# jpreprocess/jbonsai

Hardware: AMD Instinct MI355X
Metric: 48 kHz PCM samples/sec (whole node), batched utterances (higher is better)
Workload: dtype f64

## Files before the change

jbonsai_amd/csrc/jb_vocoder.hip:

```cpp
#include "jb_device.h"

#include <cstdlib>
#include <cstring>

namespace jb {

__global__ void k_pitch(BatchDev bd, VocDev vd)
{
    const int b = blockIdx.y;
    const UttDev *u = bd.utt + b;
    const uint32_t t = blockIdx.x * blockDim.x + threadIdx.x;
    if (t >= u->T)
        return;
    const uint64_t f = u->frame_off + t;
    const double MAX_LF0 = 9.903487552536127, MIN_LF0 = 2.995732273553991;
    auto pitch_of = [&](double l) {
        if (l == kNoData)
            return 0.0;
        const double cl = l < MIN_LF0 ? MIN_LF0 : (l > MAX_LF0 ? MAX_LF0 : l);
        return (double)vd.fs / exp(cl);
    };
    const double p = pitch_of(vd.lf0[f]);
    const double prevp = t > 0 ? pitch_of(vd.lf0[f - 1]) : 0.0;
    vd.pitch[f] = p;
// ... 479 lines not shown
    if (vd.pitch[f] != 0.0) {
        const unsigned long long pm = vd.pmask[f * (uint64_t)nblk + (uint64_t)(i / bs)];
        x = ((pm >> (i % bs)) & 1ull) ? sqrt(fma((double)i, vd.pinc[f], vd.cur_start[f])) : 0.0;
    } else {
        x = vd.noise[(uint64_t)vd.uv_before[f] * (uint64_t)fp + (uint64_t)i];
    }
    if (vd.exc)
        vd.exc[base * (uint64_t)fp + n] = x;
    vd.xin[base * (uint64_t)fp + n] = x;
}

constexpr int kExw = 4;
constexpr int kExwHalo = 32;
constexpr int kExwQ = (256 + kExwHalo) / kExw;

constexpr int kN4Group = 4;
template <int NLPF>
__device__ __forceinline__ bool exc_pulse_free(const VocDev &vd, const int fp, const long n0,
                                               const double *__restrict__ tc, const double *__restrict__ tpp,
                                               const bool vcur, const bool vprev, const int lane,
                                               double (*ec)[kExwQ], double *ep, double *xs, double (&x)[kExw])
{
    static_assert(NLPF - 1 <= kExwHalo - 2, "history window too short");
    constexpr int kExwWin = NLPF - 1 + kExw;
    constexpr int anti = (NLPF - 1) / 2;
    constexpr int HQ = kExwHalo / kExw;
    const int i0 = lane * kExw;
    const bool own = i0 < fp;
    double ck[NLPF];
#pragma unroll
    for (int k = 0; k < NLPF; k++)
        ck[k] = tc[k];
    const double tpv = lane < NLPF ? tpp[lane] : 0.0;
    const long nl = own ? n0 + i0 : n0;
    const double2 nva = *reinterpret_cast<const double2 *>(vd.noise + nl);
    const double2 nvb = *reinterpret_cast<const double2 *>(vd.noise + nl + 2);
    double xi[kExw];
#pragma unroll
    for (int r = 0; r < kExw; r++) {
        const long q = nl + r - anti;
        const double v = vd.noise[q < 0 ? 0 : q];
        xi[r] = q < 0 ? 0.0 : v;
    }
    const long nt = n0 - kExwHalo + i0;
    const bool has_tail = lane < HQ && nt >= 0;
    const long ntc = has_tail ? nt : n0;
    const double2 tla = *reinterpret_cast<const double2 *>(vd.noise + ntc);
    const double2 tlb = *reinterpret_cast<const double2 *>(vd.noise + ntc + 2);
    const double nv[kExw] = {nva.x, nva.y, nvb.x, nvb.y};
#pragma unroll
    for (int r = 0; r < kExw; r++)
        x[r] = xi[r];
    if (vcur) {
        if (lane < HQ) {
#pragma unroll
            for (int r = 0; r < kExw; r++)
                ec[r][lane] = 0.0;
        }
        if (own) {
#pragma unroll
            for (int r = 0; r < kExw; r++)
                ec[r][HQ + lane] = 0.0 - nv[r];
        }
    }
    if (vprev) {
        if (lane < HQ) {
            const double tl[kExw] = {tla.x, tla.y, tlb.x, tlb.y};
#pragma unroll
            for (int r = 0; r < kExw; r++)
                ep[i0 + r] = has_tail ? 0.0 - tl[r] : 0.0;
        } else if (lane < 2 * HQ) {
#pragma unroll
            for (int r = 0; r < kExw; r++)
                ep[i0 + r] = 0.0;
        }
    }
    __builtin_amdgcn_fence(__ATOMIC_RELEASE, "wavefront");
    __builtin_amdgcn_wave_barrier();
    __builtin_amdgcn_fence(__ATOMIC_ACQUIRE, "wavefront");
    if (vcur && own) {
        constexpr int G = kN4Group;
#pragma unroll
        for (int k0 = 0; k0 < NLPF; k0 += G) {
            const int k1 = k0 + G - 1 < NLPF - 1 ? k0 + G - 1 : NLPF - 1;
            const int lo = NLPF - 1 - k1;
            double wg[G + kExw - 1];
#pragma unroll
            for (int c = 0; c < G + kExw - 1; c++) {
                const int idx = lo + c;
                if (idx < kExwWin) {
                    if (idx >= NLPF - 1) {
                        wg[c] = 0.0 - nv[idx - (NLPF - 1)];
                    } else {
                        const int o = idx + kExwHalo - (NLPF - 1);
                        wg[c] = ec[o & (kExw - 1)][lane + (o >> 2)];
                    }
                } else {
                    wg[c] = 0.0;
                }
            }
#pragma unroll
            for (int k = k0; k <= k1; k++) {
#pragma unroll
                for (int r = 0; r < kExw; r++)
                    x[r] = fma(wg[NLPF - 1 + r - k - lo], ck[k], x[r]);
            }
        }
    }
    if (vprev) {
        if (own && i0 < kExwHalo) {
#pragma unroll
            for (int r = 0; r < kExw; r++)
                xs[i0 + r] = x[r];
        }
        __builtin_amdgcn_fence(__ATOMIC_RELEASE, "wavefront");
        __builtin_amdgcn_wave_barrier();
        __builtin_amdgcn_fence(__ATOMIC_ACQUIRE, "wavefront");
        {
            double tk[NLPF];
#pragma unroll
            for (int k = 1; k < NLPF; k++) {
                const int lo = __builtin_amdgcn_readlane(__double2loint(tpv), k);
                const int hi = __builtin_amdgcn_readlane(__double2hiint(tpv), k);
                tk[k] = __hiloint2double(hi, lo);
            }
            if (lane < NLPF - 1 && lane < fp) {
                double xv = xs[lane];
#pragma unroll
                for (int k = 1; k < NLPF; k++)
                    xv = fma(ep[lane - k + kExwHalo], tk[k], xv);
                xs[lane] = xv;
            }
        }
        __builtin_amdgcn_fence(__ATOMIC_RELEASE, "wavefront");
        __builtin_amdgcn_wave_barrier();
        __builtin_amdgcn_fence(__ATOMIC_ACQUIRE, "wavefront");
        if (own && i0 < kExwHalo) {
#pragma unroll
            for (int r = 0; r < kExw; r++)
                x[r] = xs[i0 + r];
        }
    }
    return own;
}

template <int NLPF>
__global__ __launch_bounds__(256) void k_exc_classify(BatchDev bd, VocDev vd)
{
    const int b = blockIdx.y;
    const UttDev *u = bd.utt + b;
    const int wv = threadIdx.x >> 6, lane = threadIdx.x & 63;
    const uint32_t T = u->T;
    const uint32_t fr0 = (blockIdx.x * 4u + (uint32_t)wv) * 64u;
    if (blockIdx.x * 256u >= T)
        return;
    __shared__ uint32_t wcount[4], wbase;
    const uint64_t base = u->frame_off;
    unsigned long long canon = 0ull;
    bool canon64 = false;
    if (!vd.exc_no_table && vd.lpf_canon) {
        const long fa = (long)fr0 - 1 + lane;
        const bool ina = fa >= 0 && fa < (long)T;
        const uint8_t ca = vd.lpf_canon[base + (uint64_t)(ina ? fa : 0)];
        const long fb = (long)fr0 + 63;
        const uint8_t cb = vd.lpf_canon[base + (uint64_t)(fb < (long)T ? fb : 0)];
        canon = __ballot(ina && ca != 0);
        canon64 = fb < (long)T && cb != 0;
    } else if (!vd.exc_no_table) {
        const int half = lane >> 5, k = lane & 31;
        const bool tap = k < NLPF;
        const double cref = vd.lpf[tap ? k : 0];
        double v[33];
#pragma unroll
        for (int s = 0; s < 33; s++) {
            const long fr = (long)fr0 - 1 + 2 * s + half;
            const bool in = tap && fr >= 0 && fr < (long)T;
            v[s] = vd.lpf[in ? (base + (uint64_t)fr) * (uint64_t)NLPF + (uint64_t)k : (uint64_t)(tap ? k : 0)];
            if (!(fr >= 0 && fr < (long)T))
                v[s] = __longlong_as_double(~__double_as_longlong(cref));
        }
#pragma unroll
        for (int s = 0; s < 33; s++)
            asm volatile("" : "+v"(v[s]));
#pragma unroll
        for (int s = 0; s < 33; s++) {
            const bool eq = !tap || __double_as_longlong(v[s]) == __double_as_longlong(cref);
            const unsigned long long m = __ballot(eq);
            const bool ea = (uint32_t)m == 0xFFFFFFFFu, eb = (uint32_t)(m >> 32) == 0xFFFFFFFFu;
            if (s < 32)
                canon |= ((unsigned long long)ea << (2 * s)) | ((unsigned long long)eb << (2 * s + 1));
            else
                canon64 = ea;
        }
    }
    const uint32_t fr = fr0 + (uint32_t)lane;
    const bool in = fr < T;
    const uint64_t f = base + (in ? fr : 0u);
    const bool vcur = in && vd.voiced[f] != 0;
    const bool vprev = in && fr > 0 && vd.voiced[f - 1] != 0;
    const bool ccur = lane == 63 ? canon64 : ((canon >> (lane + 1)) & 1ull) != 0;
    const bool cprev = ((canon >> lane) & 1ull) != 0;
    uint32_t code = 0;
    if (!vd.exc_no_table && !vcur && !vprev && fr >= 1)
        code = 1;
    else if (!vd.exc_no_table && vcur && vprev && ccur && cprev)
        code = 2;
    if (in)
        vd.exc_src[f] = (uint8_t)code;
    const bool gen = in && code == 0;
    const unsigned long long gm = __ballot(gen);
    if (lane == 0)
        wcount[wv] = (uint32_t)__popcll(gm);
    __syncthreads();
    if (threadIdx.x == 0) {
        const uint32_t tot = wcount[0] + wcount[1] + wcount[2] + wcount[3];
        wbase = tot ? atomicAdd(vd.exc_gen_count, tot) : 0u;
    }
    __syncthreads();
    uint32_t slot0 = wbase;
    for (int w = 0; w < wv; w++)
        slot0 += wcount[w];
    if (gen) {
        const uint32_t rank = (uint32_t)__popcll(gm & ((1ull << lane) - 1ull));
        uint32_t *e = vd.exc_gen + 2 * (uint64_t)(slot0 + rank);
        e[0] = (uint32_t)b;
        e[1] = fr | (vcur ? 1u << 30 : 0u) | (vprev ? 1u << 31 : 0u);
    }
}

template <int NLPF>
__global__ __launch_bounds__(256) void k_exc_table(BatchDev bd, VocDev vd)
{
    const int wv = threadIdx.x >> 6, lane = threadIdx.x & 63;
    const uint32_t fr = (uint32_t)__builtin_amdgcn_readfirstlane((int)(blockIdx.x * 4u + (uint32_t)wv));
    if (fr == 0 || fr >= bd.maxT)
        return;
    __shared__ double ec_s[4][kExw][kExwQ];
    __shared__ double ep_s[4][2 * kExwHalo];
    __shared__ double xs_s[4][kExwHalo];
    const int fp = vd.fperiod;
    const long n0 = (long)fr * (long)fp;
    double x[kExw];
    if (!exc_pulse_free<NLPF>(vd, fp, n0, vd.lpf, vd.lpf, true, true, lane, ec_s[wv], ep_s[wv], xs_s[wv], x))
        return;
    double *o = vd.exc_tab + (uint64_t)n0 + (uint64_t)(lane * kExw);
    *reinterpret_cast<double2 *>(o) = make_double2(x[0], x[1]);
    *reinterpret_cast<double2 *>(o + 2) = make_double2(x[2], x[3]);
}

template <int NLPF>
__global__ __launch_bounds__(256) void k_exc_general(BatchDev bd, VocDev vd)
{
    const int wv = threadIdx.x >> 6, lane = threadIdx.x & 63;
    __shared__ double ec_s[4][kExw][kExwQ];
    __shared__ double ep_s[4][2 * kExwHalo];
    __shared__ double xs_s[4][kExwHalo];
    const uint32_t count = *vd.exc_gen_count;
    const uint32_t stride = gridDim.x * 4u;
    uint32_t i = blockIdx.x * 4u + (uint32_t)wv;
    if (i >= count)
        return;
    const int fp = vd.fperiod;
    uint32_t eb = vd.exc_gen[2 * (uint64_t)i], ef = vd.exc_gen[2 * (uint64_t)i + 1];
    for (; i < count; i += stride) {
        const int b = __builtin_amdgcn_readfirstlane((int)eb);
        const uint32_t efu = (uint32_t)__builtin_amdgcn_readfirstlane((int)ef);
        const uint32_t inext = i + stride < count ? i + stride : i;
        eb = vd.exc_gen[2 * (uint64_t)inext];
        ef = vd.exc_gen[2 * (uint64_t)inext + 1];
        const uint32_t fr = efu & 0x3FFFFFFFu;
        const bool vcur = (efu >> 30 & 1u) != 0, vprev = (efu >> 31) != 0;
        const uint64_t base = bd.utt[b].frame_off;
        const uint64_t f = base + fr;
        const uint64_t fprev = fr > 0 ? f - 1 : f;
        const long n0 = (long)fr * (long)fp;
        double x[kExw];
        const bool own = exc_pulse_free<NLPF>(vd, fp, n0, lpf_row(vd, f, NLPF), lpf_row(vd, fprev, NLPF),
                                              vcur, vprev, lane, ec_s[wv], ep_s[wv], xs_s[wv], x);
        if (own) {
            const uint64_t o = base * (uint64_t)fp + (uint64_t)n0 + (uint64_t)(lane * kExw);
            *reinterpret_cast<double2 *>(vd.xin + o) = make_double2(x[0], x[1]);
            *reinterpret_cast<double2 *>(vd.xin + o + 2) = make_double2(x[2], x[3]);
            if (vd.exc) {
                *reinterpret_cast<double2 *>(vd.exc + o) = make_double2(x[0], x[1]);
                *reinterpret_cast<double2 *>(vd.exc + o + 2) = make_double2(x[2], x[3]);
            }
        }
        __builtin_amdgcn_fence(__ATOMIC_RELEASE, "wavefront");
        __builtin_amdgcn_wave_barrier();
        __builtin_amdgcn_fence(__ATOMIC_ACQUIRE, "wavefront");
    }
}

__device__ __forceinline__ double readlane_f64(double v, int lane)
{
    int lo = __builtin_amdgcn_readlane(__double2loint(v), lane);
    int hi = __builtin_amdgcn_readlane(__double2hiint(v), lane);
    return __hiloint2double(hi, lo);
}

constexpr int kFixFrames = 8;

template <int NLPF>
__global__ __launch_bounds__(256) void k_excite_fix(BatchDev bd, VocDev vd)
{
    const int b = blockIdx.y;
    const UttDev *u = bd.utt + b;
    const int wv = threadIdx.x >> 6, lane = threadIdx.x & 63;
    const uint32_t T = u->T;
    const uint64_t base = u->frame_off;
    const int fp = vd.fperiod, bs = vd.bs, nblk = vd.nblk;
    constexpr int H = NLPF - 1;
    __shared__ double tap_s[4][2][NLPF];
    double(*tap2)[NLPF] = tap_s[wv];
    static_assert(kFixFrames * 4 <= 32, "one lane per (frame, mask word), twice");
    const int s0 = lane * kExw;
    const bool own = s0 < fp;
    const bool blk_rows = bs % kExw == 0 && bs % 2 == 0 && nblk <= 4;
    int myblk = 0;
    for (int q = 1; q < nblk; q++)
        myblk += s0 >= q * bs ? 1 : 0;
    const int tail0 = fp - H;
    unsigned long long mword = 0ull;
    uint32_t vfl = 0, codev = 0;
    uint32_t cnv = 0;
    {
        const int half = lane >> 5, jf = (lane & 31) / 4, q = lane & 3;
        const long frl = (long)((blockIdx.x * (uint32_t)kFixFrames + (uint32_t)jf) * 4u + (uint32_t)wv) - half;
        if (frl >= 0 && frl < (long)T) {
            if (q == 0)
                vfl = vd.voiced[base + (uint64_t)frl];
            if (q == 1 && half == 0 && vd.exc_src)
                codev = vd.exc_src[base + (uint64_t)frl];
            if (q == 2 && vd.lpf_sparse)
                cnv = vd.lpf_canon[base + (uint64_t)frl];
            if (q < nblk)
                mword = vd.pmask[(base + (uint64_t)frl) * (uint64_t)nblk + (uint64_t)q];
        }
        const uint32_t vq = (uint32_t)__builtin_amdgcn_update_dpp(0, (int)vfl, 0x00, 0xf, 0xf, true);
        if (!vq)
            mword = 0ull;
        if (half) {
            const int qt = tail0 / bs, lo = tail0 - qt * bs;
            if (q < qt)
                mword = 0ull;
            else if (q == qt && lo > 0)
                mword &= ~0ull << lo;
        }
    }
    const unsigned long long nz = __ballot(mword != 0ull);
    auto words_of = [&](int jf) -> uint32_t {
        return (uint32_t)((nz >> (32 + 4 * jf)) & 0xFull) | ((uint32_t)((nz >> (4 * jf)) & 0xFull) << 4);
    };
    auto each_pulse = [&](int jf, uint32_t m8, auto fn) {
        while (m8) {
            const int idx = __builtin_ctz(m8);
            m8 &= m8 - 1u;
            const int ownf = idx >> 2, q = idx & 3;
            const int src = (ownf ? 0 : 32) + jf * 4 + q;
            const uint32_t wl = (uint32_t)__builtin_amdgcn_readlane((int)(uint32_t)mword, src);
            const uint32_t wh = (uint32_t)__builtin_amdgcn_readlane((int)(uint32_t)(mword >> 32), src);
            unsigned long long w = ((unsigned long long)wh << 32) | wl;
            while (w) {
                const int j = __builtin_ctzll(w);
                w &= w - 1ull;
                fn(ownf ? q * bs + j : q * bs + j - fp, ownf, q * bs + j);
            }
        }
    };
#ifndef JB_FIX_GROUP
#define JB_FIX_GROUP 4
#endif
    constexpr int kFixGroup = JB_FIX_GROUP;
    static_assert(kFixFrames % kFixGroup == 0, "whole groups");
    for (int j0 = 0; j0 < kFixFrames; j0 += kFixGroup) {
        bool work[kFixGroup], touched[kFixGroup], from_tab[kFixGroup];
        uint32_t bmask[kFixGroup];
        double tv[kFixGroup], pv[kFixGroup], x[kFixGroup][kExw];
#pragma unroll
        for (int g = 0; g < kFixGroup; g++) {
            const int jf = j0 + g;
            const uint32_t fr = (uint32_t)__builtin_amdgcn_readfirstlane(
                (int)((blockIdx.x * (uint32_t)kFixFrames + (uint32_t)jf) * 4u + (uint32_t)wv));
            work[g] = touched[g] = from_tab[g] = false;
            bmask[g] = 0;
            tv[g] = pv[g] = 0.0;
#pragma unroll
            for (int r = 0; r < kExw; r++)
                x[g][r] = 0.0;
            if (fr >= T)
                continue;
            const uint64_t f = base + fr;
            const uint32_t m8 = words_of(jf);
            if (!m8)
                continue;
            const bool any_p = (m8 & 0xFu) != 0, any_c = (m8 >> 4) != 0;
            bool tch = false;
            each_pulse(jf, m8, [&](int p, int, int) { tch = tch || (s0 + kExw - 1 >= p && s0 <= p + H); });
            from_tab[g] = (__builtin_amdgcn_readlane((int)codev, 4 * jf + 1) & 3) == 2;
            work[g] = true;
            bool in_blk = true;
            if (from_tab[g] && blk_rows) {
                uint32_t bm = 0;
                for (int q = 0; q < nblk; q++)
                    if (__ballot(tch && own && myblk == q))
                        bm |= 1u << q;
                bmask[g] = bm;
                in_blk = ((bm >> myblk) & 1u) != 0;
            }
            touched[g] = (tch || (from_tab[g] && in_blk)) && own;
            {
                const int hw = lane >> 5, k = lane & 31;
                const uint32_t cn_c = (uint32_t)__builtin_amdgcn_readlane((int)cnv, 4 * jf + 2);
                const uint32_t cn_p = (uint32_t)__builtin_amdgcn_readlane((int)cnv, 32 + 4 * jf + 2);
                if (k < NLPF && (hw ? any_c : any_p))
                    tv[g] = vd.lpf[((hw ? cn_c : cn_p) ? 0ull : f - 1 + (uint64_t)hw) * (uint64_t)NLPF + (uint64_t)k];
                if (lane < 4 && ((lane >> 1) ? any_c : any_p)) {
                    const uint64_t ff = f - 1 + (uint64_t)(lane >> 1);
                    pv[g] = (lane & 1) ? vd.pinc[ff] : vd.cur_start[ff];
                }
            }
            if (touched[g]) {
                const double *src = from_tab[g] ? vd.exc_tab + ((uint64_t)fr * (uint64_t)fp + (uint64_t)s0)
                                                : vd.xin + (f * (uint64_t)fp + (uint64_t)s0);
                const double2 xa = *reinterpret_cast<const double2 *>(src);
                const double2 xb = *reinterpret_cast<const double2 *>(src + 2);
                x[g][0] = xa.x;
                x[g][1] = xa.y;
                x[g][2] = xb.x;
                x[g][3] = xb.y;
            }
        }
#pragma unroll
        for (int g = 0; g < kFixGroup; g++) {
            if (!work[g])
                continue;
            const int jf = j0 + g;
            const uint32_t fr = (uint32_t)__builtin_amdgcn_readfirstlane(
                (int)((blockIdx.x * (uint32_t)kFixFrames + (uint32_t)jf) * 4u + (uint32_t)wv));
            const uint64_t f = base + fr;
            __builtin_amdgcn_fence(__ATOMIC_RELEASE, "wavefront");
            __builtin_amdgcn_wave_barrier();
            if ((lane & 31) < NLPF)
                tap2[lane >> 5][lane & 31] = tv[g];
            const double cs_p = readlane_f64(pv[g], 0), pi_p = readlane_f64(pv[g], 1);
            const double cs_c = readlane_f64(pv[g], 2), pi_c = readlane_f64(pv[g], 3);
            __builtin_amdgcn_fence(__ATOMIC_RELEASE, "wavefront");
            __builtin_amdgcn_wave_barrier();
            __builtin_amdgcn_fence(__ATOMIC_ACQUIRE, "wavefront");
            each_pulse(jf, words_of(jf), [&](int p, int gsel, int i) {
                const double amp = sqrt(gsel ? fma((double)i, pi_c, cs_c) : fma((double)i, pi_p, cs_p));
#pragma unroll
                for (int r = 0; r < kExw; r++) {
                    const int k = s0 + r - p;
                    const bool in = k >= 0 && k <= H;
                    const double tk = tap2[gsel][in ? k : 0];
                    if (in)
                        x[g][r] = fma(amp, tk, x[g][r]);
                }
            });
            if (touched[g]) {
                const uint64_t o = f * (uint64_t)fp + (uint64_t)s0;
                *reinterpret_cast<double2 *>(vd.xin + o) = make_double2(x[g][0], x[g][1]);
                *reinterpret_cast<double2 *>(vd.xin + o + 2) = make_double2(x[g][2], x[g][3]);
                if (vd.exc) {
                    *reinterpret_cast<double2 *>(vd.exc + o) = make_double2(x[g][0], x[g][1]);
                    *reinterpret_cast<double2 *>(vd.exc + o + 2) = make_double2(x[g][2], x[g][3]);
                }
            }
            if (from_tab[g] && lane == 0)
                vd.exc_src[f] = blk_rows ? (uint8_t)(2u | (bmask[g] << 4)) : (uint8_t)0;
        }
    }
}

template <int CTRL>
__device__ __forceinline__ double dpp_f64(double v)
{
    int lo = __double2loint(v), hi = __double2hiint(v);
    lo = __builtin_amdgcn_update_dpp(0, lo, CTRL, 0xf, 0xf, true);
    hi = __builtin_amdgcn_update_dpp(0, hi, CTRL, 0xf, 0xf, true);
    return __hiloint2double(hi, lo);
}
constexpr int DPP_ROW_SHR1 = 0x111, DPP_ROW_SHR2 = 0x112, DPP_ROW_SHR4 = 0x114,
              DPP_ROW_SHR8 = 0x118, DPP_WAVE_SHR1 = 0x138, DPP_ROW_BCAST15 = 0x142;


__device__ __forceinline__ int pcm_i16(double v)
{
    v = fmin(v, 32767.0);
    v = fmax(v, -32768.0);
    return (int)v;
}
__device__ __forceinline__ uint32_t pcm_i16x2(double a, double b)
{
    return ((uint32_t)pcm_i16(a) & 0xffffu) | ((uint32_t)pcm_i16(b) << 16);
}

struct ScanCoef {
    double c1, c2, c4, c8, cb;
};

__device__ __forceinline__ double seg_scan(double v, const ScanCoef &k)
{
    v = fma(k.c1, dpp_f64<DPP_ROW_SHR1>(v), v);
    v = fma(k.c2, dpp_f64<DPP_ROW_SHR2>(v), v);
    v = fma(k.c4, dpp_f64<DPP_ROW_SHR4>(v), v);
    v = fma(k.c8, dpp_f64<DPP_ROW_SHR8>(v), v);
    v = fma(k.cb, dpp_f64<DPP_ROW_BCAST15>(v), v);
    return v;
}

__device__ __forceinline__ double ipow(double x, int n)
{
    double r = 1.0;
    for (int i = 0; i < n; i++)
        r *= x;
    return r;
}

__device__ __constant__ double kPPade[6] = {1.00000000000, 0.49993910000, 0.11070980000,
                                            0.01369984000, 0.00095648530, 0.00003041721};

__host__ __device__ inline int voc_state_doubles(int tpl) { return 64 * tpl + 64 + 16; }

template <int TPL>
__global__ __launch_bounds__(256) void k_vocoder(BatchDev bd, VocDev vd, const VocWork *__restrict__ work,
                                                 uint32_t n_items)
{
    const uint32_t item = blockIdx.x * 4u + (threadIdx.x >> 6);
    if (item >= n_items)
        return;
    const VocWork wk = work[item];
    const int b = (int)wk.utt;
    const uint32_t T = bd.utt[b].T;
    const uint32_t t_begin = wk.t_start, t_out = wk.t_out;
    uint32_t t_end = wk.t_end;
    if (t_end > T)
        t_end = T;
    if (t_begin >= t_end)
        return;
    const int lane = threadIdx.x & 63;
    const uint64_t base = bd.utt[b].frame_off;
    const int nmcp = vd.nmcp, fp = vd.fperiod, bs = vd.bs, nblk = vd.nblk;
    const int M = nmcp - 1;
    const double a = wave_uniform(voc_alpha(vd, (uint32_t)b)), iaa = 1.0 - a * a,
                 vol = wave_uniform(voc_volume(vd, (uint32_t)b));

    const int s = lane / kGroups, g = lane % kGroups;
    const bool active = lane < kPade * kGroups;
    const bool head = active && g == 0;
    const double kappa = ipow(-a, TPL);
    ScanCoef kc, ks;
    {
        const int r16 = lane & 15;
        auto ok = [&](int sh) { return active && g >= sh && r16 >= sh; };
        kc.c1 = ok(1) ? ipow(kappa, 1) : 0.0;
        kc.c2 = ok(2) ? ipow(kappa, 2) : 0.0;
        kc.c4 = ok(4) ? ipow(kappa, 4) : 0.0;
        kc.c8 = ok(8) ? ipow(kappa, 8) : 0.0;
        const int rowstart = lane & ~15, segstart = s * kGroups;
        const bool straddle = active && rowstart > 0 && segstart < rowstart;
        kc.cb = straddle ? ipow(kappa, lane - rowstart + 1) : 0.0;
        ks.c1 = kc.c1 != 0.0 ? 1.0 : 0.0;
        ks.c2 = kc.c2 != 0.0 ? 1.0 : 0.0;
        ks.c4 = kc.c4 != 0.0 ? 1.0 : 0.0;
        ks.c8 = kc.c8 != 0.0 ? 1.0 : 0.0;
        ks.cb = straddle ? 1.0 : 0.0;
    }
    const double nh = (active && !head) ? 1.0 : 0.0;
    const double hmask = (head && s > 0) ? 1.0 : 0.0;
    const double l0mask = (lane == 0) ? 1.0 : 0.0;
    const double Pl = active ? kPPade[s + 1] : 0.0;
    int tapj[TPL];
    bool dotv[TPL];
#pragma unroll
    for (int k = 0; k < TPL; k++) {
        tapj[k] = g * TPL + k + 1;
        dotv[k] = active && tapj[k] >= 2 && tapj[k] <= M;
    }

    double d[TPL], cd[TPL], cdinc[TPL], ctgt[TPL];
#pragma unroll
    for (int k = 0; k < TPL; k++)
        d[k] = 0.0;
    double ulane = 0.0;
    double e11[6], e12[6];
#pragma unroll
    for (int i = 0; i < 6; i++)
        e11[i] = e12[i] = 0.0;
    if (wk.load_state) {
        const double *sp = wk.load_state;
#pragma unroll
        for (int k = 0; k < TPL; k++)
            d[k] = sp[64 * k + lane];
        ulane = sp[64 * TPL + lane];
#pragma unroll
        for (int i = 0; i < 6; i++) {
            e11[i] = sp[64 * TPL + 64 + i];
            e12[i] = sp[64 * TPL + 70 + i];
        }
    }

    auto save_state = [&](double *sp) {
#pragma unroll
        for (int k = 0; k < TPL; k++)
            sp[64 * k + lane] = d[k];
        sp[64 * TPL + lane] = ulane;
        if (lane == 0) {
#pragma unroll
            for (int i = 0; i < 6; i++) {
                sp[64 * TPL + 64 + i] = e11[i];
                sp[64 * TPL + 70 + i] = e12[i];
            }
        }
    };

    for (uint32_t t = t_begin; t < t_end; t++) {
        const uint64_t f = base + t;
        const bool emit = t >= t_out;
        if (t == t_out && t_out > t_begin && wk.save_warm)
            save_state(wk.save_warm);
        if (t == t_out + vd.ckpt_frames && wk.save_ckpt)
            save_state(wk.save_ckpt);
        if (vd.ckpt2_frames && t == t_out + vd.ckpt2_frames && wk.save_ckpt2)
            save_state(wk.save_ckpt2);
        const double *bcur = vd.bcoef + f * (uint64_t)nmcp;
        const double *bprev = (t > 0) ? bcur - nmcp : (vd.bfirst ? vd.bfirst + (uint64_t)b * (uint64_t)nmcp : bcur);
#pragma unroll
        for (int k = 0; k < TPL; k++) {
            double c0v = dotv[k] ? bprev[tapj[k]] : 0.0;
            double c1v = dotv[k] ? bcur[tapj[k]] : 0.0;
            cd[k] = c0v;
            ctgt[k] = c1v;
            cdinc[k] = (c1v - c0v) / (double)fp;
        }
        double c1 = bprev[1];
        const double c1inc = (bcur[1] - c1) / (double)fp;
        double gain = exp(bprev[0]);
        const double gq = exp((bcur[0] - bprev[0]) / (double)fp);
        for (int q = 0; q < nblk; q++) {
            const int i0 = q * bs;
            const uint64_t n0 = (uint64_t)t * (uint64_t)fp + (uint64_t)i0;
            const int blen = min(bs, fp - i0);
            const double xin = lane < blen ? exc_block_ptr(vd, base, t, exc_code(vd, base, t), q)[i0 + lane] : 0.0;
            double ob = 0.0;
            for (int i = 0; i < blen; i++) {
                double x = readlane_f64(xin, i) * gain;
                gain *= gq;
                {
                    double out = 0.0;
#pragma unroll
                    for (int ii = 5; ii >= 1; ii--) {
                        e11[ii] = fma(iaa, e12[ii - 1], a * e11[ii]);
                        e12[ii] = e11[ii] * c1;
                        const double v = e12[ii] * kPPade[ii];
                        x += (ii & 1) ? v : -v;
                        out += v;
                    }
                    e12[0] = x;
                    x += out;
                }
                double loc = d[0];
#pragma unroll
                for (int k = 1; k < TPL; k++)
                    loc = fma(-a, loc, d[k]);
                double I = fma(kappa, ulane, loc);
                I = seg_scan(I, kc);
                double r = fma(nh, dpp_f64<DPP_WAVE_SHR1>(I), ulane);
#pragma unroll
                for (int k = 0; k < TPL; k++) {
                    const double rn = fma(-a, r, d[k]);
                    d[k] = fma(a, rn, r);
                    r = rn;
                }
                double yl = cd[0] * d[0];
#pragma unroll
                for (int k = 1; k < TPL; k++)
                    yl = fma(cd[k], d[k], yl);
                const double Y = seg_scan(yl, ks);
                const double Yp = Y * Pl;
                const double v1 = readlane_f64(Yp, 11), v2 = readlane_f64(Yp, 23),
                             v3 = readlane_f64(Yp, 35), v4 = readlane_f64(Yp, 47),
                             v5 = readlane_f64(Yp, 59);
                x += v5;
                x -= v4;
                x += v3;
                x -= v2;
                x += v1;
                double out = v5;
                out += v4;
                out += v3;
                out += v2;
                out += v1;
                ulane = fma(hmask, dpp_f64<DPP_WAVE_SHR1>(Y), l0mask * x);
                x += out;
#pragma unroll
                for (int k = 0; k < TPL; k++)
                    cd[k] += cdinc[k];
                c1 += c1inc;
                ob = (lane == i) ? x * vol : ob;
            }
            if (lane < blen && emit) {
                if (vd.pcm16)
                    vd.pcm16[base * (uint64_t)fp + n0 + (uint64_t)lane] = (int16_t)pcm_i16(ob);
                else
                    vd.pcm[base * (uint64_t)fp + n0 + (uint64_t)lane] = ob;
            }
        }
        (void)ctgt;
    }

    if (wk.save_end)
        save_state(wk.save_end);
}

template <int TPL, int ITEMS>
__global__ __launch_bounds__(128 * ITEMS) void k_vocoder_pair(BatchDev bd, VocDev vd, const VocWork *__restrict__ work,
                                                              uint32_t n_items)
{
    __shared__ double xbuf[ITEMS][2][64];
    __shared__ double obuf[ITEMS][2][64];
    __shared__ uint32_t nblocks_sh[ITEMS];
    const int wv = threadIdx.x >> 6, lane = threadIdx.x & 63;
    const int slot = wv % ITEMS;
    const bool producer = wv >= ITEMS;
    const uint32_t item = blockIdx.x * (uint32_t)ITEMS + (uint32_t)slot;
    const int fp = vd.fperiod, bs = vd.bs, nblk = vd.nblk, nmcp = vd.nmcp;
    VocWork wk{};
    uint32_t t_begin = 0, t_end = 0, t_out = 0;
    int b = 0;
    if (item < n_items) {
        wk = work[item];
        b = (int)wk.utt;
        t_begin = wk.t_start;
        t_out = wk.t_out;
        t_end = min(wk.t_end, bd.utt[b].T);
        if (t_begin >= t_end)
            t_begin = t_end = 0;
    }
    const uint32_t NB = (t_end - t_begin) * (uint32_t)nblk;
    if (!producer && lane == 0)
        nblocks_sh[slot] = NB;
    __syncthreads();
    uint32_t NBmax = 0;
#pragma unroll
    for (int j = 0; j < ITEMS; j++)
        NBmax = max(NBmax, nblocks_sh[j]);
    const uint64_t base = NB ? bd.utt[b].frame_off : 0;
    const double a = wave_uniform(voc_alpha(vd, (uint32_t)b)), iaa = 1.0 - a * a,
                 vol = wave_uniform(voc_volume(vd, (uint32_t)b));
    double *const xb = &xbuf[slot][0][0];
    double *const ob = &obuf[slot][0][0];

    if (producer) {
        double e11[6], e12[6];
#pragma unroll
        for (int i = 0; i < 6; i++)
            e11[i] = e12[i] = 0.0;
        if (NB && wk.load_state) {
#pragma unroll
            for (int i = 0; i < 6; i++) {
                e11[i] = wk.load_state[64 * TPL + 64 + i];
// ... 521 lines not shown
            };
            cv[1] = 0.0;
#pragma unroll
            for (int j = 1; j <= M; j++) {
                if (j == 1)
                    wait_pair(2, 2);
                else if (j % 2 == 0 && j + 2 <= M)
                    wait_pair(j + 2, j + 4 <= M ? 1 : 0);
                if (j + 1 <= M) {
                    const int sq = (j - 1) % kLtPf;
                    cv[j + 1] = fma(fi, cq[sq].y, cq[sq].x);
                    if (j + 5 <= M)
                        JB_LDS_RD(cq[sq], j + 5);
                }
                const double cj = cv[j];
                if constexpr (NS == 1) {
                    double rn0;
                    if (j <= 2) {
                        asm volatile("v_fma_f64 %[rn0], %[na], %[r0], %[d0]\n\t"
                            "v_fma_f64 %[d0], %[a], %[rn0], %[r0]"
                            : [rn0] "=&v"(rn0), [d0] "+v"(d[0][j])
                            : [na] "s"(na), [a] "s"(a), [r0] "v"(r[0]));
                    } else if (j == 3) {
                        asm volatile("v_fma_f64 %[rn0], %[na], %[r0], %[d0]\n\t"
                            "v_mul_f64 %[y0], %[c], %[dp]\n\t"
                            "v_fma_f64 %[d0], %[a], %[rn0], %[r0]"
                            : [rn0] "=&v"(rn0), [d0] "+v"(d[0][j]), [y0] "=&v"(y[0])
                            : [na] "s"(na), [a] "s"(a), [r0] "v"(r[0]), [c] "v"(cv[j - 1]), [dp] "v"(d[0][j - 1]));
                    } else {
                        asm volatile("v_fma_f64 %[rn0], %[na], %[r0], %[d0]\n\t"
                            "v_fma_f64 %[y0], %[c], %[dp], %[y0]\n\t"
                            "v_fma_f64 %[d0], %[a], %[rn0], %[r0]"
                            : [rn0] "=&v"(rn0), [d0] "+v"(d[0][j]), [y0] "+v"(y[0])
                            : [na] "s"(na), [a] "s"(a), [r0] "v"(r[0]), [c] "v"(cv[j - 1]), [dp] "v"(d[0][j - 1]));
                    }
                    r[0] = rn0;
                    if (j == M)
                        y[0] = fma(cj, d[0][M], y[0]);
                } else {
                    double rn0, rn1;
                    if (j == 2) {
                        asm volatile("v_fma_f64 %[rn0], %[na], %[r0], %[d0]\n\t"
                            "v_fma_f64 %[rn1], %[na], %[r1], %[d1]\n\t"
                            "v_fma_f64 %[d0], %[a], %[rn0], %[r0]\n\t"
                            "v_fma_f64 %[d1], %[a], %[rn1], %[r1]\n\t"
                            "v_mul_f64 %[y0], %[c], %[d0]\n\t"
                            "v_mul_f64 %[y1], %[c], %[d1]"
                            : [rn0] "=&v"(rn0), [rn1] "=&v"(rn1), [d0] "+v"(d[0][j]), [d1] "+v"(d[1][j]),
                              [y0] "=&v"(y[0]), [y1] "=&v"(y[1])
                            : [na] "s"(na), [a] "s"(a), [r0] "v"(r[0]), [r1] "v"(r[1]), [c] "v"(cj));
                    } else if (j > 2) {
                        asm volatile("v_fma_f64 %[rn0], %[na], %[r0], %[d0]\n\t"
                            "v_fma_f64 %[rn1], %[na], %[r1], %[d1]\n\t"
                            "v_fma_f64 %[d0], %[a], %[rn0], %[r0]\n\t"
                            "v_fma_f64 %[d1], %[a], %[rn1], %[r1]\n\t"
                            "v_fma_f64 %[y0], %[c], %[d0], %[y0]\n\t"
                            "v_fma_f64 %[y1], %[c], %[d1], %[y1]"
                            : [rn0] "=&v"(rn0), [rn1] "=&v"(rn1), [d0] "+v"(d[0][j]), [d1] "+v"(d[1][j]),
                              [y0] "+v"(y[0]), [y1] "+v"(y[1])
                            : [na] "s"(na), [a] "s"(a), [r0] "v"(r[0]), [r1] "v"(r[1]), [c] "v"(cj));
                    } else {
                        asm volatile("v_fma_f64 %[rn0], %[na], %[r0], %[d0]\n\t"
                            "v_fma_f64 %[rn1], %[na], %[r1], %[d1]\n\t"
                            "v_fma_f64 %[d0], %[a], %[rn0], %[r0]\n\t"
                            "v_fma_f64 %[d1], %[a], %[rn1], %[r1]"
                            : [rn0] "=&v"(rn0), [rn1] "=&v"(rn1), [d0] "+v"(d[0][j]), [d1] "+v"(d[1][j])
                            : [na] "s"(na), [a] "s"(a), [r0] "v"(r[0]), [r1] "v"(r[1]));
                    }
                    r[0] = rn0;
                    r[1] = rn1;
                }
            }
#undef JB_LDS_RD
            double ssum, psum;
            if constexpr (NS == 2) {
                const double v1 = w1 * y[1];
                const double sb = fma(w0, y[0], v1), sa = fma(w0, y[0], db1 - v1);
                ssum = sa + dpp_f64<DPP_WAVE_SHL1>(sa + dpp_f64<DPP_WAVE_SHL1>(sa));
                psum = sb + dpp_f64<DPP_WAVE_SHL1>(sb + dpp_f64<DPP_WAVE_SHL1>(sb));
            } else {
                ssum = fold5(fma(wa, y[0], db1));
                psum = fold5(w0 * y[0]);
            }
            const double yprev = dpp_f64<DPP_WAVE_SHR1>(y[NS - 1]);
            const double xmid = x + ssum;
            x = xmid + psum;
            if constexpr (NS == 2)
                u[1] = y[0];
            u[0] = pos == 0 ? xmid : yprev;
            const double pv = x * vol;
            if (ODD)
                oB = pv;
            else
                oA = pv;
        };
        int xnext = xbs, xqn = 1;
        for (int i2 = 0; i2 < fp; i2 += 2) {
            if (i2 + 2 == xnext && xnext < fp) {
                xq = xblock(xqn);
                xqn++;
                xnext += xbs;
            }
            if (kLtWaves == 8 && i2 % kLtBalance == 0) {
                const uint32_t mine = tl * (uint32_t)fp + (uint32_t)i2;
                uint32_t theirs;
                asm volatile("ds_write_b32 %1, %2\n\t"
                             "ds_read_b32 %0, %3\n\t"
                             "s_waitcnt lgkmcnt(0)"
                             : "=v"(theirs)
                             : "v"((uint32_t)(uintptr_t)&prog[wv]), "v"(mine), "v"((uint32_t)(uintptr_t)&prog[wv ^ 4])
                             : "memory");
                if (mine > (uint32_t)__builtin_amdgcn_readfirstlane((int)theirs))
                    __builtin_amdgcn_s_setprio(0);
                else
                    __builtin_amdgcn_s_setprio(1);
            }
            sample(i2, std::false_type{});
            sample(i2 + 1, std::true_type{});
        }
        asm volatile("s_waitcnt vmcnt(0)" : "+v"(xn), "+v"(xo)::"memory");
        if (emit)
            put_pair(fp - 2);
        if (act && tl + 1 == nfr) {
            double *se_ = work[item].save_end;
            if (se_)
                save_state(se_);
        }
    }
    if (kLtWaves == 8 && lane == 0)
        prog[wv] = 0xffffffffu;
#ifdef JB_LT_STAMPS
    if (lane == 0 && stamp_w < kLtStampWaves)
        g_lt_stamp[stamp_w][1] = wall_clock64();
#endif
#ifdef JB_LT_CLOCKS
    if (clk_slot >= 0 && lane == 0) {
        g_lt_clk[clk_slot + 2] = clock64();
        g_lt_clk[clk_slot + 3] = wall_clock64();
    }
#endif
}

__device__ __forceinline__ bool voc_state_differs(const double *__restrict__ a, const double *__restrict__ r,
                                                  int nfilt, int ntaps, double tol, int lane, double *md_out,
                                                  double *mr_out)
{
    double md = 0.0, mr = 0.0;
    const int urow = nfilt - 76;
    const int tpl = urow / 64;
    for (int k = lane; k < nfilt; k += 64) {
        if (ntaps < 0) {
        } else if (k < urow) {
            const int ln = k & 63, kk = k >> 6;
            if (ln >= kGroups * kPade || (ln % kGroups) * tpl + kk >= ntaps)
                continue;
        } else if (k < urow + 64 && ((k - urow) % kGroups != 0 || (k - urow) >= kGroups * kPade)) {
            continue;
        }
        const double x = a[k], y = r[k];
        md = fmax(md, fabs(x - y));
        mr = fmax(mr, fabs(y));
        if (!(x == x) || !(y == y))
            md = 1e300;
    }
    for (int o = 32; o > 0; o >>= 1) {
        md = fmax(md, __shfl_xor(md, o));
        mr = fmax(mr, __shfl_xor(mr, o));
    }
    *md_out = md;
    *mr_out = mr;
    return md > tol * mr && md > 1e-300;
}

__global__ __launch_bounds__(64) void k_voc_verify(const VocWork *__restrict__ work, uint32_t n_items,
                                                    int nfilt , int ntaps, double tol,
                                                    uint8_t *bad, uint32_t *n_bad)
{
    const uint32_t i = blockIdx.x;
    if (i >= n_items)
        return;
    const VocWork wk = work[i];
    const int lane = threadIdx.x;
    if (!wk.save_warm || i == 0) {
        if (lane == 0)
            bad[i] = 0;
        return;
    }
    double md, mr;
    const bool isbad = voc_state_differs(wk.save_warm, work[i - 1].save_end, nfilt, ntaps, tol, lane, &md, &mr);
    if (lane == 0) {
        bad[i] = isbad;
        if (isbad)
            atomicAdd(n_bad, 1u);
#ifdef JB_VERIFY_DEBUG
        if (isbad)
            printf("handoff item %u utt %u t_out %u: max|diff| %.3e max|state| %.3e ratio %.3e\n", i, wk.utt,
                   wk.t_out, md, mr, md / mr);
#endif
    }
}

__global__ __launch_bounds__(64) void k_voc_verify_pairs(const double *const *__restrict__ pairs, uint32_t n_pairs,
                                                          int nfilt, int ntaps, double tol, uint8_t *bad,
                                                          uint32_t *n_bad)
{
    const uint32_t i = blockIdx.x;
    if (i >= n_pairs)
        return;
    const int lane = threadIdx.x;
    double md, mr;
    const bool isbad = voc_state_differs(pairs[2 * i], pairs[2 * i + 1], nfilt, ntaps, tol, lane, &md, &mr);
    if (lane == 0) {
        bad[i] = isbad;
        if (isbad)
            atomicAdd(n_bad, 1u);
#ifdef JB_VERIFY_DEBUG
        printf("state pair %u: max|diff| %.3e max|state| %.3e %s\n", i, md, mr, isbad ? "FAIL" : "ok");
#endif
    }
}

static int tpl_for(int nmcp)
{
    int M = nmcp - 1;
    int tpl = (M + kGroups - 1) / kGroups;
    return tpl < 1 ? 1 : tpl;
}

int vocoder_state_doubles(int nmcp) { return voc_state_doubles(tpl_for(nmcp)); }

hipError_t launch_pitch(const BatchDev &bd, const VocDev &vd, hipStream_t stream)
{
    if (bd.B == 0 || bd.maxT == 0)
        return hipSuccess;
    dim3 grid((bd.maxT + 255) / 256, bd.B), block(256);
    hipLaunchKernelGGL(k_pitch, grid, block, 0, stream, bd, vd);
    return hipGetLastError();
}

hipError_t launch_mc2b(const BatchDev &bd, const VocDev &vd, hipStream_t stream)
{
    if (bd.B == 0 || bd.maxT == 0)
        return hipSuccess;
    dim3 grid((bd.maxT + kMc2bFrames - 1) / kMc2bFrames, bd.B), block(kMc2bFrames);
    hipLaunchKernelGGL(k_mc2b, grid, block, 0, stream, bd, vd);
    return hipGetLastError();
}

static int current_device_cus()
{
    static int cus_of[64] = {0};
    int dev = 0, cus = 0;
    if (hipGetDevice(&dev) != hipSuccess || dev < 0 || dev >= 64)
        return 0;
    if ((cus = cus_of[dev]) == 0) {
        if (hipDeviceGetAttribute(&cus, hipDeviceAttributeMultiprocessorCount, dev) != hipSuccess || cus <= 0)
            return 0;
        cus_of[dev] = cus;
    }
    return cus;
}

bool excite_is_split(const VocDev &vd)
{
    return vd.fperiod % kExw == 0 && vd.fperiod <= 256 && vd.fperiod >= kExwHalo && (vd.nlpf == 31 || vd.nlpf == 15) &&
           vd.nblk <= 4 && vd.fperiod % vd.bs == 0;
}

hipError_t launch_excite_noise(const BatchDev &bd, const VocDev &vd, hipStream_t stream)
{
    if (bd.B == 0 || bd.maxT == 0 || !excite_is_split(vd))
        return hipSuccess;
    if (!vd.exc_src || !vd.exc_gen || !vd.exc_gen_count || !vd.exc_tab)
        return hipErrorInvalidValue;
    hipError_t e = hipMemsetAsync(vd.exc_gen_count, 0, sizeof(uint32_t), stream);
    if (e != hipSuccess)
        return e;
    const dim3 block(256);
    const dim3 gcls((bd.maxT + 255) / 256, bd.B), gtab((bd.maxT + 3) / 4);
    constexpr size_t pad = 32 * 1024;
    int cus = current_device_cus();
    if (cus <= 0)
        cus = 256;
    const dim3 ggen((unsigned)(3 * cus));
    if (vd.nlpf == 31) {
        hipLaunchKernelGGL(k_exc_classify<31>, gcls, block, 0, stream, bd, vd);
        if (!vd.exc_no_table)
            hipLaunchKernelGGL(k_exc_table<31>, gtab, block, 0, stream, bd, vd);
        JB_DBG_SKIP_IF(4, hipLaunchKernelGGL(k_exc_general<31>, ggen, block, pad, stream, bd, vd));
    } else {
        hipLaunchKernelGGL(k_exc_classify<15>, gcls, block, 0, stream, bd, vd);
        if (!vd.exc_no_table)
            hipLaunchKernelGGL(k_exc_table<15>, gtab, block, 0, stream, bd, vd);
        hipLaunchKernelGGL(k_exc_general<15>, ggen, block, pad, stream, bd, vd);
    }
    return hipGetLastError();
}

hipError_t launch_excite(const BatchDev &bd, const VocDev &vd, hipStream_t stream)
{
    if (bd.B == 0 || bd.maxT == 0)
        return hipSuccess;
    if (excite_is_split(vd)) {
        dim3 gfix((bd.maxT + 4 * kFixFrames - 1) / (4 * kFixFrames), bd.B), block(256);
        if (vd.nlpf == 31)
            JB_DBG_SKIP_IF(8, hipLaunchKernelGGL(k_excite_fix<31>, gfix, block, 0, stream, bd, vd));
        else
            hipLaunchKernelGGL(k_excite_fix<15>, gfix, block, 0, stream, bd, vd);
        return hipGetLastError();
    }
    const uint64_t maxN = (uint64_t)bd.maxT * (uint64_t)vd.fperiod;
    dim3 grid((unsigned)((maxN + kExcBlock - 1) / kExcBlock), bd.B), block(kExcBlock);
    if (vd.nlpf == 0) {
        if (!vd.uv_before)
            return hipErrorInvalidValue;
        hipLaunchKernelGGL(k_uv_scan, dim3(bd.B), dim3(64), 0, stream, bd, vd);
        hipLaunchKernelGGL(k_excite_nolpf, grid, block, 0, stream, bd, vd);
        return hipGetLastError();
    }
    if (excite_fits_staged(vd))
        hipLaunchKernelGGL(k_excite, grid, block, 0, stream, bd, vd);
    else
        hipLaunchKernelGGL(k_excite_any, grid, block, (size_t)(kExcBlock + vd.nlpf - 1) * sizeof(double), stream, bd, vd);
    return hipGetLastError();
}

constexpr unsigned kPulseQueueWaves = 512;
hipError_t launch_pulse(const BatchDev &bd, const VocDev &vd, hipStream_t stream)
{
    if (bd.B == 0 || bd.maxT == 0)
        return hipSuccess;
    hipLaunchKernelGGL(k_run_scan, dim3(1), dim3(256), 0, stream, bd, vd);
    JB_DBG_SKIP_IF(64, hipLaunchKernelGGL(k_pulse_queue, dim3(kPulseQueueWaves), dim3(64), 0, stream, bd, vd));
    return hipGetLastError();
}

hipError_t launch_voc_verify(const VocWork *work_dev, uint32_t n_items, int state_doubles, int ntaps, double tol,
                             uint8_t *bad, uint32_t *n_bad, hipStream_t stream)
{
    if (n_items == 0)
        return hipSuccess;
    hipLaunchKernelGGL(k_voc_verify, dim3(n_items), dim3(64), 0, stream, work_dev, n_items,
                       ntaps < 0 ? state_doubles : state_doubles - 4, ntaps, tol, bad, n_bad);
    return hipGetLastError();
}

hipError_t launch_voc_verify_pairs(const double *const *pairs_dev, uint32_t n_pairs, int state_doubles, int ntaps,
                                   double tol, uint8_t *bad, uint32_t *n_bad, hipStream_t stream)
{
    if (n_pairs == 0)
        return hipSuccess;
    hipLaunchKernelGGL(k_voc_verify_pairs, dim3(n_pairs), dim3(64), 0, stream, pairs_dev, n_pairs,
                       ntaps < 0 ? state_doubles : state_doubles - 4, ntaps, tol, bad, n_bad);
    return hipGetLastError();
}

hipError_t launch_vocoder_ls(const BatchDev &bd, const VocDev &vd, const VocWork *work_dev,
                             const uint32_t *order_dev, uint32_t n_items, int waves_per_simd, hipStream_t stream)
{
    if (n_items == 0)
        return hipSuccess;
    if ((waves_per_simd != 1 && waves_per_simd != 2) || !vocoder_ls_supported(vd.nmcp))
        return hipErrorInvalidValue;
    const int wv = 4 * waves_per_simd;
    const int code = lt_code_nm(vd.nmcp);
    const bool exact = vd.nmcp == 35 || vd.nmcp == 25;
    const uint32_t per_wg = (uint32_t)(vocoder_ls_chunks_per_wave(vd.nmcp) * wv);
    dim3 grid((n_items + per_wg - 1) / per_wg), block(64 * wv);
#define JB_LT_LAUNCH(NMc, TPLc, EX, LPCc)                                                                              \
    do {                                                                                                           \
        if (wv == 8)                                                                                               \
            hipLaunchKernelGGL((k_vocoder_lt<NMc, TPLc, 8, EX, LPCc>), grid, block, 0, stream, bd, vd, work_dev,      \
                               order_dev, n_items);                                                                \
        else                                                                                                       \
            hipLaunchKernelGGL((k_vocoder_lt<NMc, TPLc, 4, EX, LPCc>), grid, block, 0, stream, bd, vd, work_dev,      \
                               order_dev, n_items);                                                                \
    } while (0)
    if (exact && code == 35)
        JB_LT_LAUNCH(35, 3, true, 3);
    else if (exact && code == 25)
        JB_LT_LAUNCH(25, 2, true, 3);
    else if (code == 25)
        JB_LT_LAUNCH(25, 2, false, 3);
    else if (code == 31)
        JB_LT_LAUNCH(31, 3, false, 3);
    else if (code == 35)
        JB_LT_LAUNCH(35, 3, false, 3);
    else if (code == 41)
        JB_LT_LAUNCH(41, 4, false, 5);
    else if (code == 51)
        JB_LT_LAUNCH(51, 5, false, 5);
    else
        JB_LT_LAUNCH(61, 5, false, 5);
#undef JB_LT_LAUNCH
#ifdef JB_LT_STAMPS
    if (const char *path = getenv("JB_LT_STAMPS_FILE")) {
        static unsigned long long st[kLtStampWaves][4];
        hipStreamSynchronize(stream);
        const unsigned nw = std::min<unsigned>(kLtStampWaves, grid.x * (unsigned)wv);
        if (hipMemcpyFromSymbol(st, HIP_SYMBOL(g_lt_stamp), sizeof st) == hipSuccess)
            if (FILE *f = fopen(path, "w")) {
                fprintf(f, "# wave start_10ns end_10ns hw_id xcc frames   (k_vocoder_lt, %u waves, %d per workgroup)\n", nw, wv);
                for (unsigned w = 0; w < nw; w++)
                    fprintf(f, "%u %llu %llu %llu %llu %llu\n", w, st[w][0], st[w][1], st[w][2] & 0xffffffffull,
                            st[w][2] >> 32, st[w][3]);
                fclose(f);
            }
        unsigned long long t0 = ~0ull, last[16] = {0};
        for (unsigned w = 0; w < nw; w++)
            if (st[w][0] && st[w][0] < t0)
                t0 = st[w][0];
        for (unsigned w = 0; w < nw; w++)
            last[(st[w][2] >> 32) & 15] = std::max(last[(st[w][2] >> 32) & 15], st[w][1]);
        fprintf(stderr, "k_vocoder_lt last wave end per XCD, ms:");
        for (int x = 0; x < 8; x++)
            fprintf(stderr, " %.2f", last[x] ? (double)(last[x] - t0) / 1e5 : 0.0);
        fprintf(stderr, "\n");
    }
#endif
#ifdef JB_LT_CLOCKS
    {
        unsigned long long c[8];
        hipStreamSynchronize(stream);
        if (hipMemcpyFromSymbol(c, HIP_SYMBOL(g_lt_clk), sizeof c) == hipSuccess)
            for (int k = 0; k < 8; k += 4) {
                const double us = (double)(c[k + 3] - c[k + 1]) / 100.0;
                fprintf(stderr, "k_vocoder_lt wave %d: %.3f ms, %.0f shader-clock ticks = %.3f GHz\n", k / 4, us / 1e3,
                        (double)(c[k + 2] - c[k]), (double)(c[k + 2] - c[k]) / us / 1e3);
            }
    }
#endif
    return hipGetLastError();
}

hipError_t launch_vocoder(const BatchDev &bd, const VocDev &vd, const VocWork *work_dev, uint32_t n_items,
                          hipStream_t stream, bool fixed_form)
{
    if (n_items == 0)
        return hipSuccess;
    if (vd.stage > 0)
        return launch_vocoder_mglsa(bd, vd, work_dev, n_items, stream);
    dim3 grid((n_items + 3) / 4), block(256);
    const int cus = fixed_form ? 0 : current_device_cus();
    const char *nop = getenv("JB_NO_PAIR_KERNEL");
    if (cus > 0 && n_items <= 2u * (uint32_t)cus && !(nop && nop[0] == '1')) {
        const dim3 gp((n_items + 1) / 2);
        switch (tpl_for(vd.nmcp)) {
#define JB_PAIR_CASE(T)                                                                                            \
    case T:                                                                                                        \
        hipLaunchKernelGGL((k_vocoder_pair<T, 2>), gp, dim3(256), 0, stream, bd, vd, work_dev, n_items);            \
        break;
            JB_PAIR_CASE(1)
            JB_PAIR_CASE(2)
            JB_PAIR_CASE(3)
            JB_PAIR_CASE(4)
            JB_PAIR_CASE(5)
            JB_PAIR_CASE(6)
#undef JB_PAIR_CASE
        default:
            return hipErrorInvalidValue;
        }
        return hipGetLastError();
    }
    if (cus > 0 && n_items <= 4u * (uint32_t)cus && !nop) {
        const dim3 gp((n_items + 3) / 4);
        switch (tpl_for(vd.nmcp)) {
#define JB_PAIR_CASE(T)                                                                                            \
    case T:                                                                                                        \
        hipLaunchKernelGGL((k_vocoder_pair<T, 4>), gp, dim3(512), 0, stream, bd, vd, work_dev, n_items);            \
        break;
            JB_PAIR_CASE(1)
            JB_PAIR_CASE(2)
            JB_PAIR_CASE(3)
            JB_PAIR_CASE(4)
            JB_PAIR_CASE(5)
            JB_PAIR_CASE(6)
#undef JB_PAIR_CASE
        default:
            return hipErrorInvalidValue;
        }
        return hipGetLastError();
    }
    switch (tpl_for(vd.nmcp)) {
    case 1:
        hipLaunchKernelGGL(k_vocoder<1>, grid, block, 0, stream, bd, vd, work_dev, n_items);
        break;
    case 2:
        hipLaunchKernelGGL(k_vocoder<2>, grid, block, 0, stream, bd, vd, work_dev, n_items);
        break;
    case 3:
        hipLaunchKernelGGL(k_vocoder<3>, grid, block, 0, stream, bd, vd, work_dev, n_items);
        break;
    case 4:
        hipLaunchKernelGGL(k_vocoder<4>, grid, block, 0, stream, bd, vd, work_dev, n_items);
        break;
    case 5:
        hipLaunchKernelGGL(k_vocoder<5>, grid, block, 0, stream, bd, vd, work_dev, n_items);
        break;
    case 6:
        hipLaunchKernelGGL(k_vocoder<6>, grid, block, 0, stream, bd, vd, work_dev, n_items);
        break;
    default:
        return hipErrorInvalidValue;
    }
    return hipGetLastError();
}

}
```

Before: 20.17 billion.

## Cache pulse positions during first scan and reorder excite-fix grid utterance-fastest

```diff
diff --git a/jbonsai_amd/csrc/jb_vocoder.hip b/jbonsai_amd/csrc/jb_vocoder.hip
--- a/jbonsai_amd/csrc/jb_vocoder.hip
+++ b/jbonsai_amd/csrc/jb_vocoder.hip
@@ -805,12 +805,15 @@
 constexpr int kFixFrames = 8;
 
 template <int NLPF>
-__global__ __launch_bounds__(256) void k_excite_fix(BatchDev bd, VocDev vd)
-{
-    const int b = blockIdx.y;
+__global__ __launch_bounds__(256) void k_excite_fix(BatchDev bd, VocDev vd, int utt_fastest)
+{
+    const int b = utt_fastest ? blockIdx.x : blockIdx.y;
+    const uint32_t fblk = utt_fastest ? blockIdx.z * gridDim.y + blockIdx.y : blockIdx.x;
     const UttDev *u = bd.utt + b;
     const int wv = threadIdx.x >> 6, lane = threadIdx.x & 63;
     const uint32_t T = u->T;
+    if ((uint64_t)fblk * (uint64_t)(4 * kFixFrames) >= (uint64_t)T)
+        return;
     const uint64_t base = u->frame_off;
     const int fp = vd.fperiod, bs = vd.bs, nblk = vd.nblk;
     constexpr int H = NLPF - 1;
@@ -829,7 +832,7 @@
     uint32_t cnv = 0;
     {
         const int half = lane >> 5, jf = (lane & 31) / 4, q = lane & 3;
-        const long frl = (long)((blockIdx.x * (uint32_t)kFixFrames + (uint32_t)jf) * 4u + (uint32_t)wv) - half;
+        const long frl = (long)((fblk * (uint32_t)kFixFrames + (uint32_t)jf) * 4u + (uint32_t)wv) - half;
         if (frl >= 0 && frl < (long)T) {
             if (q == 0)
                 vfl = vd.voiced[base + (uint64_t)frl];
@@ -867,7 +870,7 @@
             while (w) {
                 const int j = __builtin_ctzll(w);
                 w &= w - 1ull;
-                fn(ownf ? q * bs + j : q * bs + j - fp, ownf, q * bs + j);
+                fn(ownf ? q * bs + j : q * bs + j - fp);
             }
         }
     };
@@ -876,17 +879,25 @@
 #endif
     constexpr int kFixGroup = JB_FIX_GROUP;
     static_assert(kFixFrames % kFixGroup == 0, "whole groups");
+    constexpr int kPkBits = 9, kPkMax = 64 / kPkBits, kPkBias = 32;
+    constexpr int kPovMax = 256 + H - kPkMax;
+    static_assert(H <= kPkBias && 256 + kPkBias <= (1 << kPkBits), "a position fits its field");
+    __shared__ uint16_t pov_s[4][kFixGroup][kPovMax];
     for (int j0 = 0; j0 < kFixFrames; j0 += kFixGroup) {
         bool work[kFixGroup], touched[kFixGroup], from_tab[kFixGroup];
         uint32_t bmask[kFixGroup];
+        unsigned long long ppk[kFixGroup];
+        int pn[kFixGroup];
         double tv[kFixGroup], pv[kFixGroup], x[kFixGroup][kExw];
 #pragma unroll
         for (int g = 0; g < kFixGroup; g++) {
             const int jf = j0 + g;
             const uint32_t fr = (uint32_t)__builtin_amdgcn_readfirstlane(
-                (int)((blockIdx.x * (uint32_t)kFixFrames + (uint32_t)jf) * 4u + (uint32_t)wv));
+                (int)((fblk * (uint32_t)kFixFrames + (uint32_t)jf) * 4u + (uint32_t)wv));
             work[g] = touched[g] = from_tab[g] = false;
             bmask[g] = 0;
+            ppk[g] = 0ull;
+            pn[g] = 0;
             tv[g] = pv[g] = 0.0;
 #pragma unroll
             for (int r = 0; r < kExw; r++)
@@ -899,7 +910,20 @@
                 continue;
             const bool any_p = (m8 & 0xFu) != 0, any_c = (m8 >> 4) != 0;
             bool tch = false;
-            each_pulse(jf, m8, [&](int p, int, int) { tch = tch || (s0 + kExw - 1 >= p && s0 <= p + H); });
+            {
+                unsigned long long pk = 0ull;
+                int n = 0;
+                each_pulse(jf, m8, [&](int p) {
+                    tch = tch || (s0 + kExw - 1 >= p && s0 <= p + H);
+                    const uint32_t code = (uint32_t)(p + kPkBias);
+                    pk |= (unsigned long long)(n < kPkMax ? code : 0u) << ((kPkBits * n) & 63);
+                    if (n >= kPkMax && lane == 0 && n - kPkMax < kPovMax)
+                        pov_s[wv][g][n - kPkMax] = (uint16_t)code;
+                    n++;
+                });
+                ppk[g] = pk;
+                pn[g] = n;
+            }
             from_tab[g] = (__builtin_amdgcn_readlane((int)codev, 4 * jf + 1) & 3) == 2;
             work[g] = true;
             bool in_blk = true;
@@ -940,7 +964,7 @@
                 continue;
             const int jf = j0 + g;
             const uint32_t fr = (uint32_t)__builtin_amdgcn_readfirstlane(
-                (int)((blockIdx.x * (uint32_t)kFixFrames + (uint32_t)jf) * 4u + (uint32_t)wv));
+                (int)((fblk * (uint32_t)kFixFrames + (uint32_t)jf) * 4u + (uint32_t)wv));
             const uint64_t f = base + fr;
             __builtin_amdgcn_fence(__ATOMIC_RELEASE, "wavefront");
             __builtin_amdgcn_wave_barrier();
@@ -951,7 +975,9 @@
             __builtin_amdgcn_fence(__ATOMIC_RELEASE, "wavefront");
             __builtin_amdgcn_wave_barrier();
             __builtin_amdgcn_fence(__ATOMIC_ACQUIRE, "wavefront");
-            each_pulse(jf, words_of(jf), [&](int p, int gsel, int i) {
+            auto add_pulse = [&](int p) {
+                const int gsel = p >= 0 ? 1 : 0;
+                const int i = gsel ? p : p + fp;
                 const double amp = sqrt(gsel ? fma((double)i, pi_c, cs_c) : fma((double)i, pi_p, cs_p));
 #pragma unroll
                 for (int r = 0; r < kExw; r++) {
@@ -961,7 +987,22 @@
                     if (in)
                         x[g][r] = fma(amp, tk, x[g][r]);
                 }
-            });
+            };
+            {
+                const int n = pn[g], nreg = n < kPkMax ? n : kPkMax;
+                unsigned long long pk = ppk[g];
+                for (int k = 0; k < nreg; k++) {
+                    add_pulse((int)((uint32_t)pk & ((1u << kPkBits) - 1u)) - kPkBias);
+                    pk >>= kPkBits;
+                }
+                for (int k0 = kPkMax; k0 < n; k0 += 64) {
+                    const int e = k0 - kPkMax + lane;
+                    const int v = e < kPovMax ? (int)pov_s[wv][g][e] : 0;
+                    const int m = n - k0 < 64 ? n - k0 : 64;
+                    for (int k = 0; k < m; k++)
+                        add_pulse(__builtin_amdgcn_readlane(v, k) - kPkBias);
+                }
+            }
             if (touched[g]) {
                 const uint64_t o = f * (uint64_t)fp + (uint64_t)s0;
                 *reinterpret_cast<double2 *>(vd.xin + o) = make_double2(x[g][0], x[g][1]);
@@ -2089,11 +2130,19 @@
     if (bd.B == 0 || bd.maxT == 0)
         return hipSuccess;
     if (excite_is_split(vd)) {
-        dim3 gfix((bd.maxT + 4 * kFixFrames - 1) / (4 * kFixFrames), bd.B), block(256);
+        const unsigned nfb = (bd.maxT + 4 * kFixFrames - 1) / (4 * kFixFrames);
+        const char *ord = getenv("JB_EXCITE_FIX_ORDER");
+        const int utt_fastest = !(ord && ord[0] == 'f');
+        constexpr unsigned kGridMax = 65535u;
+        if ((unsigned)bd.B > kGridMax || (nfb + kGridMax - 1) / kGridMax > kGridMax)
+            return hipErrorInvalidValue;
+        const unsigned gy = nfb < kGridMax ? nfb : kGridMax;
+        const dim3 gfix = utt_fastest ? dim3((unsigned)bd.B, gy, (nfb + gy - 1) / gy) : dim3(nfb, (unsigned)bd.B);
+        const dim3 block(256);
         if (vd.nlpf == 31)
-            JB_DBG_SKIP_IF(8, hipLaunchKernelGGL(k_excite_fix<31>, gfix, block, 0, stream, bd, vd));
+            JB_DBG_SKIP_IF(8, hipLaunchKernelGGL(k_excite_fix<31>, gfix, block, 0, stream, bd, vd, utt_fastest));
         else
-            hipLaunchKernelGGL(k_excite_fix<15>, gfix, block, 0, stream, bd, vd);
+            hipLaunchKernelGGL(k_excite_fix<15>, gfix, block, 0, stream, bd, vd, utt_fastest);
         return hipGetLastError();
     }
     const uint64_t maxN = (uint64_t)bd.maxT * (uint64_t)vd.fperiod;
```

New measurement: 20.16 billion, median of 2. About the same (-0.0%).
